# antonilo/unsupervised_detection

Hardware: NVIDIA H100
Metric: frame-pairs/sec adversarial train step 256x448 (higher is better)
Workload: dtype bf16

## Files before the change

### include/cis_b200.h

```cpp
#ifndef CIS_B200_H_
#define CIS_B200_H_
#include <stdint.h>
#include <stddef.h>

#ifdef __cplusplus
extern "C" {
#endif

typedef void* cis_stream_t;

enum { CIS_OK = 0, CIS_ERR_BAD_ARG = 1, CIS_ERR_UNSUPPORTED = 2, CIS_ERR_CUDA = 3 };
enum { CIS_ACT_NONE = 0, CIS_ACT_ELU = 1, CIS_ACT_LEAKY = 2 };
enum { CIS_MAX_TAPS = 49, CIS_MAX_SRC = 4 };

typedef struct {
  const void* ptr;
  int32_t pitch;
  int32_t c_off;
  int32_t chunks;
  int32_t n_mod;
} CisSrc;

typedef struct {
  int32_t N, H, W;
// ... 31 lines not shown
  int32_t ey, ex;
  int32_t splits;
  float* sk_scratch;
  int32_t* sk_counters;
  int32_t nph;
  int32_t ph_tap[5];
  int32_t sk_cluster;
  int32_t nsub;
  struct {
    int32_t tap0, ntaps;
    int32_t hoy, hox;
    int32_t OH, OW, oa, ob;
    const void* wpack;
  } sub[4];
  int32_t nwg;
} CisConv;

typedef struct {
  int32_t N, H, W, OH, OW, sh, sw, ntaps;
  int16_t dh[CIS_MAX_TAPS];
  int16_t dw[CIS_MAX_TAPS];
  int32_t nsrc;
  CisSrc src[CIS_MAX_SRC];
  const void* g;
  int32_t g_pitch, g_coff, g_chunks;
  float* dwp;
  int32_t Cout;
  int32_t K_pad;
  int32_t splits;
  int32_t tma;
// ... 115 lines not shown
```

### unsupervised_detection_b200/_lib.py

```python
import ctypes as C
import os

_HERE = os.path.dirname(os.path.abspath(__file__))
LIB_PATH = os.path.join(_HERE, os.environ.get('CIS_LIB_NAME', 'libcis_b200.so'))

MAX_TAPS, MAX_SRC = 49, 4
ACT_NONE, ACT_ELU, ACT_LEAKY = 0, 1, 2


class CisSrc(C.Structure):
    _fields_ = [('ptr', C.c_void_p), ('pitch', C.c_int32), ('c_off', C.c_int32), ('chunks', C.c_int32), ('n_mod', C.c_int32)]


class CisParamJob(C.Structure):
    _fields_ = [('kind', C.c_int32), ('i', C.c_int32 * 8), ('n', C.c_int64), ('p', C.c_void_p * 8)]


JOB_PACK, JOB_PACK_TILED, JOB_UNPACK, JOB_BN_FOLD, JOB_BN_CHAIN = range(5)


class CisSub(C.Structure):
    _fields_ = [('tap0', C.c_int32), ('ntaps', C.c_int32), ('hoy', C.c_int32), ('hox', C.c_int32), ('OH', C.c_int32), ('OW', C.c_int32),
                ('oa', C.c_int32), ('ob', C.c_int32), ('wpack', C.c_void_p)]

# ... 4 lines not shown
                ('dh', C.c_int16 * MAX_TAPS), ('dw', C.c_int16 * MAX_TAPS),
                ('nsrc', C.c_int32), ('src', CisSrc * MAX_SRC),
                ('wpack', C.c_void_p), ('K_pad', C.c_int32), ('BN', C.c_int32), ('n_tiles', C.c_int32),
                ('bias', C.c_void_p), ('act', C.c_int32), ('alpha', C.c_float),
                ('DH', C.c_int32), ('DW', C.c_int32), ('osh', C.c_int32), ('osw', C.c_int32), ('oa', C.c_int32), ('ob', C.c_int32),
                ('out', C.c_void_p), ('out_pitch', C.c_int32), ('out_coff', C.c_int32), ('out_ch', C.c_int32),
                ('outf', C.c_void_p), ('outf_pitch', C.c_int32), ('outf_coff', C.c_int32), ('outf_ch', C.c_int32),
                ('add_pre', C.c_void_p), ('add_pre_pitch', C.c_int32), ('add_pre_coff', C.c_int32),
                ('addf_pre', C.c_void_p), ('addf_pitch', C.c_int32), ('addf_coff', C.c_int32),
                ('add_post', C.c_void_p), ('add_post_pitch', C.c_int32), ('add_post_coff', C.c_int32),
                ('mode', C.c_int32),
                ('halo', C.c_int32), ('dil', C.c_int32), ('MT', C.c_int32), ('hoy', C.c_int32), ('hox', C.c_int32),
                ('ey', C.c_int32), ('ex', C.c_int32),
                ('splits', C.c_int32), ('sk_scratch', C.c_void_p), ('sk_counters', C.c_void_p),
                ('nph', C.c_int32), ('ph_tap', C.c_int32 * 5), ('sk_cluster', C.c_int32),
                ('nsub', C.c_int32), ('sub', CisSub * 4), ('nwg', C.c_int32)]


class CisWgrad(C.Structure):
    _fields_ = [('N', C.c_int32), ('H', C.c_int32), ('W', C.c_int32), ('OH', C.c_int32), ('OW', C.c_int32),
                ('sh', C.c_int32), ('sw', C.c_int32), ('ntaps', C.c_int32),
                ('dh', C.c_int16 * MAX_TAPS), ('dw', C.c_int16 * MAX_TAPS),
                ('nsrc', C.c_int32), ('src', CisSrc * MAX_SRC),
                ('g', C.c_void_p), ('g_pitch', C.c_int32), ('g_coff', C.c_int32), ('g_chunks', C.c_int32),
                ('dwp', C.c_void_p), ('Cout', C.c_int32), ('K_pad', C.c_int32), ('splits', C.c_int32), ('tma', C.c_int32),
                ('nh', C.c_int32), ('nwg', C.c_int32)]


_i32, _i64, _f32, _p, _u64 = C.c_int32, C.c_int64, C.c_float, C.c_void_p, C.c_uint64

_PROTOS = {
# ... 83 lines not shown
```

### unsupervised_detection_b200/csrc/conv_igemm.cu

```cuda
#include "ptx.cuh"
#include "../../include/cis_b200.h"
#include "common.cuh"
#include <cuda.h>
#include <stdlib.h>
#include <string.h>


namespace cis {

#ifdef CIS_TRACE
__device__ unsigned long long* g_trace = nullptr;
__device__ int g_trace_cap = 0;
#define CIS_TRACE_AT(slot)                                                                                         \
  do {                                                                                                             \
    if (g_trace && blockIdx.x == 0 && blockIdx.y == 0 && blockIdx.z == 0 && (slot) < g_trace_cap) g_trace[(slot)] = clock64(); \
  } while (0)
#else
#define CIS_TRACE_AT(slot) ((void)0)
#endif

static constexpr int kBM = 128;
static constexpr int kBK = 64;
static constexpr int kAStage = kBM * 128;
static constexpr int kThreads = 256;
// ... 522 lines not shown
__device__ __forceinline__ void halo_issue_any(const int nk16, float (&acc)[MTM][BN], const uint32_t hlo, const uint32_t blo, const uint32_t* s_aoff,
                                               const int gt, const int MT, const uint32_t ahi, const uint32_t bhi, const uint32_t a_mstep,
                                               const uint32_t a_half, const bool first) {
  static_assert(MTM >= 1 && MTM <= 4, "1..4 stacked tiles");
  if (MT == 1) halo_issue_nk<1>(nk16, acc, hlo, blo, s_aoff, gt, ahi, bhi, a_mstep, a_half, first);
  else if constexpr (MTM >= 2) {
    if (MT == 2) halo_issue_nk<2>(nk16, acc, hlo, blo, s_aoff, gt, ahi, bhi, a_mstep, a_half, first);
    else if constexpr (MTM >= 3) {
      if (MT == 3) halo_issue_nk<3>(nk16, acc, hlo, blo, s_aoff, gt, ahi, bhi, a_mstep, a_half, first);
      else if constexpr (MTM >= 4) halo_issue_nk<4>(nk16, acc, hlo, blo, s_aoff, gt, ahi, bhi, a_mstep, a_half, first);
    }
  }
  wg_wait<0>();
}

template <int BN, int NWG>
__global__ void __launch_bounds__(HaloCfg<BN, NWG>::kThreads, 1) conv_halo_kernel(const __grid_constant__ CisConv p, const int halo_stage_bytes, const int BS, const int NHS,
                                                        const __grid_constant__ HaloMaps maps, const int use_tma, const int G) {
  using Cfg = HaloCfg<BN, NWG>;
  constexpr int kBStage = BN * 128;
  constexpr int kHMmaWarp_ = Cfg::kMmaWarp, kHThreads_ = Cfg::kThreads;
  extern __shared__ uint8_t smem_raw[];
  __shared__ uint64_t bars[2 * 2 + 2 * kHaloMaxBStages + 1];
  __shared__ uint32_t s_aoff[CIS_MAX_TAPS];
  __shared__ SrcS s_src[CIS_MAX_SRC];

  const int tid = threadIdx.x, warp = tid >> 5, lane = tid & 31;
  const int MT = p.MT, MTC = NWG * MT, d = p.dil;
  const int nph = p.nph > 1 ? p.nph : 1;
  const int Wh = 8 + p.ex, Hh = 16 * MTC + p.ey, HP = Wh * Hh;
  const uint32_t stage_bytes = (uint32_t)G * kBStage;
  const uint32_t tile_base = (smem_u32(smem_raw) + 1023u) & ~1023u;
  const uint32_t h_base = tile_base;
  const uint32_t b_base = tile_base + NHS * halo_stage_bytes;
  int* pixtab = reinterpret_cast<int*>(smem_raw + (b_base + BS * stage_bytes - smem_u32(smem_raw)));
  const uint32_t bar_hfull = smem_u32(&bars[0]), bar_hempty = smem_u32(&bars[2]);
  const uint32_t bar_bfull = smem_u32(&bars[4]), bar_bempty = smem_u32(&bars[4 + kHaloMaxBStages]);
  const uint32_t bar_accum = smem_u32(&bars[4 + 2 * kHaloMaxBStages]);

  const bool grouped = p.nsub > 1;
  const int tap0 = grouped ? p.sub[blockIdx.z].tap0 : 0, ntaps = grouped ? p.sub[blockIdx.z].ntaps : p.ntaps;
  const int hoy = grouped ? p.sub[blockIdx.z].hoy : p.hoy, hox = grouped ? p.sub[blockIdx.z].hox : p.hox;
  const int OHs = grouped ? p.sub[blockIdx.z].OH : p.OH, OWs = grouped ? p.sub[blockIdx.z].OW : p.OW;
  const int oa = grouped ? p.sub[blockIdx.z].oa : p.oa, ob = grouped ? p.sub[blockIdx.z].ob : p.ob;
  const void* const wpack = grouped ? p.sub[blockIdx.z].wpack : p.wpack;
  const int Hp0 = (OHs + d - 1) / d, Wp0 = (OWs + d - 1) / d;
  const int tiles_x = (Wp0 + 7) / 8, tiles_y = (Hp0 + 16 * MTC - 1) / (16 * MTC);
  if (grouped && (int)blockIdx.x >= tiles_x * tiles_y * p.N) return;
  int bid = blockIdx.x;
  const int tx = bid % tiles_x; bid /= tiles_x;
  const int ty = bid % tiles_y; bid /= tiles_y;
  const int ph = bid % (d * d);
  const int n = bid / (d * d);
  const int pa = ph / d, pb = ph % d;
  const int ny = blockIdx.y;
  int m_chunks = 0;
  for (int i = 0; i < p.nsrc; ++i) m_chunks += p.src[i].chunks;
  const int nchunks_all = (m_chunks + 7) / 8;
  const int nsplit = (!grouped && p.splits > 1) ? p.splits : 1;
  const int cper = (nchunks_all + nsplit - 1) / nsplit;
  const int cc_lo = grouped ? 0 : blockIdx.z * cper;
  const int nchunks = min(cper, nchunks_all - cc_lo);
  __shared__ __align__(16) float s_bias[BN];
  pdl_launch_dependents();

  if (tid < ntaps) s_aoff[tid] = (uint32_t)((p.dh[tap0 + tid] * Wh + p.dw[tap0 + tid]) * 8);
  if (tid < p.nsrc) {
    s_src[tid].ptr = reinterpret_cast<const __nv_bfloat16*>(p.src[tid].ptr);
    s_src[tid].pitch = p.src[tid].pitch;
    s_src[tid].c_off = p.src[tid].c_off;
    s_src[tid].chunks = p.src[tid].chunks;
    s_src[tid].n_mod = p.src[tid].n_mod;
  }
  for (int q = tid; q < (use_tma ? 0 : HP); q += kHThreads_) {
    const int hy = q / Wh, hx = q - hy * Wh;
    const int gy = ty * 16 * MTC + hy + hoy, gx = tx * 8 + hx + hox;
    const int y = pa + d * gy, x = pb + d * gx;
    pixtab[q] = (gy >= 0 && gx >= 0 && y < p.H && x < p.W) ? (y * p.W + x) : -1;
  }
  if (tid == kHMmaWarp_ * 32) {
    for (int s = 0; s < 2; ++s) {
      mbar_init(bar_hfull + 8 * s, use_tma ? 1 : 96);
      mbar_init(bar_hempty + 8 * s, NWG);
    }
    for (int s = 0; s < BS; ++s) {
      mbar_init(bar_bfull + 8 * s, 1);
      mbar_init(bar_bempty + 8 * s, NWG);
    }
    mbar_init(bar_accum, 128 * NWG);
    fence_mbar_init();
  }
  if (use_tma && tid < p.nsrc) tma_prefetch_desc(&maps.m[tid]);
  pdl_wait();
  if (tid < BN) s_bias[tid] = p.bias ? p.bias[ny * BN + tid] : 0.f;
  __syncthreads();
  if (tid == 0) CIS_TRACE_AT(0);

  if (warp < kHMmaWarp_) {
// ... 1 lines not shown
    if (use_tma) {
      if (tid == 0) {
        int hcount = 0;
        for (int vc = 0; vc < nchunks * nph; ++vc) {
          const int cc = vc / nph, ph = vc - cc * nph;
          if (nph > 1 && p.ph_tap[ph + 1] == p.ph_tap[ph]) continue;
          const int hs = hcount % NHS;
          mbar_wait(bar_hempty + 8 * hs, (uint32_t)(((hcount / NHS) & 1) ^ 1));
          ++hcount;
          int c = (cc_lo + cc) * 8, si = 0;
          while (si < p.nsrc - 1 && c >= s_src[si].chunks) {
            c -= s_src[si].chunks;
            ++si;
          }
          const int nmod = s_src[si].n_mod;
          mbar_expect_tx(bar_hfull + 8 * hs, (uint32_t)(HP * 128));
          tma_load_4d(h_base + hs * halo_stage_bytes, &maps.m[si * nph + ph], bar_hfull + 8 * hs, c * 8, pb + d * (tx * 8 + hox),
                      pa + d * (ty * 16 * MTC + hoy), nmod ? (n % nmod) : n);
        }
      }
      __syncwarp();
    } else if (warp != 2) {
      const int hid = warp == 3 ? tid - 32 : tid;
      const int j = hid & 7, pl = hid >> 3;
      for (int cc = 0; cc < nchunks; ++cc) {
        const int hs = cc % NHS;
        mbar_wait(bar_hempty + 8 * hs, (uint32_t)(((cc / NHS) & 1) ^ 1));
        const int rem = m_chunks - (cc_lo + cc) * 8;
        const int nk16 = rem >= 8 ? 4 : (rem + 1) / 2;
        const bool need = j < 2 * nk16;
        const bool cvalid = j < rem;
        int c = (cc_lo + cc) * 8 + j, si = 0;
        if (cvalid) {
// ... 196 lines not shown
  if (!valid) return;
  float v[16];
  splitk_reduce16<BN>(tile0, nsplit, r, c0, v);
  epi_chunk(p, v, ny * BN + c0, dpix);
}
static constexpr int kPThreads = 448;
static constexpr int kPMaxAccCols = 64;

template <int BN>
__global__ void __launch_bounds__(kPThreads, 1) conv_halo_persist_kernel(const __grid_constant__ CisConv p, const int halo_stage_bytes,
                                                                       const int BS, const int NHS, const int AS, const int G,
                                                                       const __grid_constant__ HaloMaps maps, const int ws) {
  constexpr int kBStage = BN * 128;
  constexpr int kMaxHS = 4;
  extern __shared__ uint8_t smem_raw[];
  __shared__ uint64_t bars[2 * kMaxHS + 2 * kHaloMaxBStages + 4];
  __shared__ uint32_t s_aoff[CIS_MAX_TAPS];
  __shared__ __align__(16) float s_bias[BN];

  const int tid = threadIdx.x, warp = tid >> 5, lane = tid & 31;
  const int MT = p.MT;
  const int Wh = 8 + p.ex, Hh = 16 * MT + p.ey, HP = Wh * Hh;
  const uint32_t stage_bytes = (uint32_t)G * kBStage;
  const uint32_t tile_base = (smem_u32(smem_raw) + 1023u) & ~1023u;
  const uint32_t acc_bytes = (uint32_t)(MT * BN) * kAccColBytes;
  const uint32_t acc_base = tile_base, h_base = tile_base + AS * acc_bytes, b_base = h_base + NHS * halo_stage_bytes;
  const uint32_t bar_hfull = smem_u32(&bars[0]), bar_hempty = smem_u32(&bars[kMaxHS]);
  const uint32_t bar_bfull = smem_u32(&bars[2 * kMaxHS]), bar_bempty = smem_u32(&bars[2 * kMaxHS + kHaloMaxBStages]);
  const uint32_t bar_tfull = smem_u32(&bars[2 * kMaxHS + 2 * kHaloMaxBStages]), bar_tempty = smem_u32(&bars[2 * kMaxHS + 2 * kHaloMaxBStages + 2]);

  const int tiles_x = (p.OW + 7) / 8, tiles_y = (p.OH + 16 * MT - 1) / (16 * MT);
  const int total = tiles_x * tiles_y * p.N;
  int m_chunks = 0;
  for (int i = 0; i < p.nsrc; ++i) m_chunks += p.src[i].chunks;
  const int nchunks = (m_chunks + 7) / 8;

  pdl_launch_dependents();
  if (tid < p.ntaps) s_aoff[tid] = (uint32_t)((p.dh[tid] * Wh + p.dw[tid]) * 8);
  if (tid == 0) {
    for (int s = 0; s < NHS; ++s) {
      mbar_init(bar_hfull + 8 * s, 1);
      mbar_init(bar_hempty + 8 * s, 1);
    }
    for (int s = 0; s < BS; ++s) {
      mbar_init(bar_bfull + 8 * s, 1);
      mbar_init(bar_bempty + 8 * s, 1);
    }
    for (int s = 0; s < AS; ++s) {
      mbar_init(bar_tfull + 8 * s, 128);
      mbar_init(bar_tempty + 8 * s, 4);
    }
    fence_mbar_init();
  }
  if (tid < p.nsrc) tma_prefetch_desc(&maps.m[tid]);
  pdl_wait();
  if (tid < BN) s_bias[tid] = p.bias ? p.bias[tid] : 0.f;
  __syncthreads();
  if (tid == 0) {
    CIS_TRACE_AT(0);
    CIS_TRACE_AT(4);
  }

  if (warp == 12) {
    if (lane == 0) {
      int hs = 0;
      uint32_t hph = 1;
      for (int w = blockIdx.x; w < total; w += gridDim.x) {
        const int tx = w % tiles_x, r1 = w / tiles_x, ty = r1 % tiles_y, n = r1 / tiles_y;
        for (int cc = 0; cc < nchunks; ++cc) {
          mbar_wait(bar_hempty + 8 * hs, hph);
          int c = cc * 8, si = 0;
          while (si < p.nsrc - 1 && c >= p.src[si].chunks) {
            c -= p.src[si].chunks;
            ++si;
          }
          int nmod = p.src[0].n_mod;
          if (si == 1) nmod = p.src[1].n_mod;
          if (si == 2) nmod = p.src[2].n_mod;
          if (si == 3) nmod = p.src[3].n_mod;
          mbar_expect_tx(bar_hfull + 8 * hs, (uint32_t)(HP * 128));
          tma_load_4d(h_base + hs * halo_stage_bytes, &maps.m[si], bar_hfull + 8 * hs, c * 8, tx * 8 + p.hox, ty * 16 * MT + p.hoy,
                      nmod ? (n % nmod) : n);
          if (++hs == NHS) {
            hs = 0;
            hph ^= 1u;
          }
        }
      }
    }
  } else if (warp == 13) {
    if (lane == 0) {
      const uint8_t* wt = reinterpret_cast<const uint8_t*>(p.wpack);
      const int per_tile = nchunks * p.ntaps;
      if (ws) {
        if ((int)blockIdx.x < total) {
          mbar_expect_tx(bar_bfull, (uint32_t)(per_tile * kBStage));
          for (int it = 0; it < per_tile; it += 8) {
// ... 571 lines not shown
                           int estride = 1, int bc = 64, CUtensorMapSwizzle swz = CU_TENSOR_MAP_SWIZZLE_128B) {
  EncodeTiledFn enc = get_encode_tiled();
  if (!enc) return false;
  const int nb = s.n_mod > 0 ? s.n_mod : N;
  const int Hq = (H - py + step - 1) / step, Wq = (W - px + step - 1) / step;
  if (Hq < 1 || Wq < 1) return false;
  cuuint64_t dims[4] = {(cuuint64_t)s.chunks * 8, (cuuint64_t)Wq, (cuuint64_t)Hq, (cuuint64_t)nb};
  cuuint64_t strides[3] = {(cuuint64_t)step * s.pitch * 2, (cuuint64_t)step * W * s.pitch * 2, (cuuint64_t)H * W * s.pitch * 2};
  cuuint32_t box[4] = {(cuuint32_t)bc, (cuuint32_t)(bw * estride), (cuuint32_t)(bh * estride), 1};
  cuuint32_t es[4] = {1, (cuuint32_t)estride, (cuuint32_t)estride, 1};
  void* base = (void*)((const char*)s.ptr + ((size_t)(py * W + px) * s.pitch + (size_t)s.c_off) * 2);
  return enc(m, CU_TENSOR_MAP_DATA_TYPE_BFLOAT16, 4, base, dims, strides, box, es, CU_TENSOR_MAP_INTERLEAVE_NONE, swz,
             CU_TENSOR_MAP_L2_PROMOTION_L2_128B, CU_TENSOR_MAP_FLOAT_OOB_FILL_NONE) == CUDA_SUCCESS;
}

#ifdef CIS_TRACE
extern "C" int cis_trace_set(unsigned long long* buf, int cap) {
  cudaError_t e = cudaMemcpyToSymbol(cis::g_trace, &buf, sizeof(buf));
  if (e == cudaSuccess) e = cudaMemcpyToSymbol(cis::g_trace_cap, &cap, sizeof(cap));
  return e == cudaSuccess ? CIS_OK : cis_set_cuda_error(e, "cis_trace_set");
}
#endif

static int g_persist_mode = -1;
extern "C" int cis_set_persist_mode(int mode) {
  g_persist_mode = mode;
  return CIS_OK;
}

template <int BN, int NWG>
static int launch_halo(const CisConv* d, cudaStream_t st) {
  const int MTC = d->MT * NWG;
  const int Wh = 8 + d->ex, Hh = 16 * MTC + d->ey, HP = Wh * Hh;
  const int halo_stage = (HP * 128 + 1023) & ~1023;
  int chunks = 0;
  for (int i = 0; i < d->nsrc; ++i) chunks += d->src[i].chunks;
  const int nchunks = (chunks + 7) / 8;
  const int nsub = d->nsub > 1 ? d->nsub : 1;
  const int nsp = (nsub == 1 && d->splits > 1) ? d->splits : 1;
  const int cper = (nchunks + nsp - 1) / nsp;
  const int nhs = cper > 1 ? 2 : 1;
  const int dd = d->dil;
  int tiles = 0, ntaps_max = d->ntaps;
  if (nsub > 1) {
    if (nsub > 4 || dd != 1 || d->splits > 1 || d->nph > 1) return cis_set_error(CIS_ERR_BAD_ARG, "cis_conv_igemm(halo): bad grouped launch");
    ntaps_max = 0;
    int tsum = 0;
    for (int i = 0; i < nsub; ++i) {
      const int t = ((d->sub[i].OW + 7) / 8) * ((d->sub[i].OH + 16 * MTC - 1) / (16 * MTC));
      if (t > tiles) tiles = t;
      if (d->sub[i].ntaps > ntaps_max) ntaps_max = d->sub[i].ntaps;
// ... 39 lines not shown
  int splits = d->splits > 1 ? d->splits : 1;
  if (splits > 1) {
    const int per = (nchunks + splits - 1) / splits;
    if ((!d->sk_scratch && !d->sk_cluster) || d->sk_counters || (splits - 1) * per >= nchunks || (d->sk_cluster && splits > 8))
      return cis_set_error(CIS_ERR_BAD_ARG, "cis_conv_igemm(halo): bad split-K setup");
  }
  dim3 grid(tiles * dd * dd * d->N, d->n_tiles, nsub > 1 ? nsub : splits);
  HaloMaps maps;
  const int nph = d->nph > 1 ? d->nph : 1;
  static const int dil_tma = getenv("CIS_DIL_TMA") ? atoi(getenv("CIS_DIL_TMA")) : 1;
  int use_tma = ((d->dil == 1 || dil_tma) && Wh * d->dil <= 256 && Hh * d->dil <= 256) ? 1 : 0;
  for (int i = 0; use_tma && i < d->nsrc - 1; ++i)
    if (d->src[i].chunks % 8) use_tma = 0;
  for (int i = 0; use_tma && i < d->nsrc; ++i) {
    if (((uintptr_t)d->src[i].ptr + (size_t)d->src[i].c_off * 2) % 16) use_tma = 0;
    for (int ph = 0; use_tma && ph < nph; ++ph)
      if (!encode_src_map(&maps.m[i * nph + ph], d->src[i], d->N, d->H, d->W, Wh, Hh, nph > 1 ? 2 : 1, ph >> 1, ph & 1, d->dil)) use_tma = 0;
  }
  if (!use_tma) memset(&maps, 0, sizeof(maps));
  if (nph > 1 && !use_tma) return cis_set_error(CIS_ERR_UNSUPPORTED, "cis_conv_igemm(halo): stride-2 phases need the TMA halo path");
  const int persist_mode = g_persist_mode >= 0 ? g_persist_mode : (getenv("CIS_PERSIST_MODE") ? atoi(getenv("CIS_PERSIST_MODE")) : 1);
  static const int p_min_tiles = getenv("CIS_PERSIST_MIN_TILES") ? atoi(getenv("CIS_PERSIST_MIN_TILES")) : 296;
  static const int p_ws_kb = getenv("CIS_PERSIST_WS_KB") ? atoi(getenv("CIS_PERSIST_WS_KB")) : 112;
  if constexpr (BN <= kPMaxAccCols && NWG == 1) {
   if (persist_mode > 0 && use_tma && d->n_tiles == 1 && splits == 1 && nph == 1 && nsub == 1 && dd == 1 && d->MT * BN <= kPMaxAccCols) {
    const int total = tiles * d->N;
    const int per_tile = nchunks * d->ntaps;
    const int acc_stage = d->MT * BN * (int)kAccColBytes;
    const int AS = 2;
    const int fixed_p = AS * acc_stage + 1024;
    const int ws_bytes = per_tile * kB;
    int p_nhs = nchunks >= 3 ? 4 : 3;
    while (p_nhs > 2 && p_nhs * halo_stage + fixed_p + (ws_bytes <= p_ws_kb * 1024 ? ws_bytes : 2 * G * kB) > 226 * 1024) --p_nhs;
    const bool ws_fits = ws_bytes <= p_ws_kb * 1024 && p_nhs * halo_stage + fixed_p + ws_bytes <= 226 * 1024;
// ... 179 lines not shown
```

### unsupervised_detection_b200/engine.py

```python
import ctypes as C
import os

import numpy as np
import torch

from . import _lib
from ._lib import CisConv, CisWgrad, CisSrc, ACT_NONE, ACT_ELU, ACT_LEAKY


def ru(x, m):
    return (x + m - 1) // m * m


def same_pad(n_in, k, s=1, d=1):
    out = -(-n_in // s)
    total = max((out - 1) * s + (k - 1) * d + 1 - n_in, 0)
    return total // 2, total - total // 2


SIDE_STREAM = True
_SIDE = {}
MULTI_PARAM_OPS = os.environ.get('CIS_MULTI_PARAM', '1') == '1'
DACT_COLSUM = os.environ.get('CIS_DACT_COLSUM', '1') == '1'
PLAN_MODEL = int(os.environ.get('CIS_PLAN_MODEL', '4'))
# ... 138 lines not shown
                    n += 1
        return n

    def extend(self, other):
        self.ops += other.ops
        self.keep += other.keep


class Act(object):

    def __init__(self, N, H, W, C, device, buf=None, c_off=0, chanmap=None, n_mod=0, dep=frozenset(), name=''):
        if chanmap is not None and not C:
            C = max(chanmap) + 1
        self.N, self.H, self.W, self.C = N, H, W, C
        self.C8 = ru(C, 8) if chanmap is None else len(chanmap)
        if buf is None:
            buf = torch.zeros(N, H, W, self.C8, dtype=torch.bfloat16, device=device)
        self.buf = buf
        self.pitch = buf.shape[-1]
        self.c_off = c_off
        self.chanmap = list(chanmap) if chanmap is not None else list(range(C)) + [-1] * (self.C8 - C)
        self.n_mod = n_mod
        self.dep = frozenset(dep)
        self.name = name
        self.grad = None
        self.grad_written = {}
        self.device = device
        self.gen_rows = None

    @property
    def ptr(self):
        return self.buf.data_ptr()
# ... 97 lines not shown
    if cout > 64:
        return 64, 2, -(-npairs // p)
    nwg = 2 if npairs > p else 1
    return nh, nwg, -(-npairs // (nwg * p))




SPLITK = int(os.environ.get('CIS_SPLITK', '2'))
SPLITK_CLUSTER = os.environ.get('CIS_SPLITK_CLUSTER', '0') == '1'
SPLITK_MAX = int(os.environ.get('CIS_SPLITK_MAX', '16'))
SPLITK_NCTA = int(os.environ.get('CIS_SPLITK_NCTA', '64'))
SPLITK_MIN_UNITS = int(os.environ.get('CIS_SPLITK_MIN_UNITS', '18'))
HALO_SKIP_THIN = int(os.environ.get('CIS_HALO_SKIP_THIN', '0'))
HALO_MIN_UTIL = float(os.environ.get('CIS_HALO_MIN_UTIL', '0.2'))


HALO_NWG = int(os.environ.get('CIS_HALO_NWG', '2'))
HALO_NWG2_COST = 0.8


def halo_nwg(d, MT, Hp0, Wp0, dil, n_tiles, ntaps, nchunks, ey, ex):
    if HALO_NWG < 2 or d.BN < 64:
        return 1
    if HALO_NWG == 2 and n_tiles == 1 and dil == 1 and MT * d.BN <= 64 and nchunks * ntaps * d.BN * 128 <= 112 * 1024:
        return 1
    tiles_x = -(-Wp0 // 8)
    ty1, ty2 = -(-Hp0 // (16 * MT)), -(-Hp0 // (32 * MT))
    HP = (8 + ex) * (32 * MT + ey)
    nhs = 2 if nchunks > 1 else 1
# ... 29 lines not shown
    splits = min(units // min_units, -(-2 * NUM_SMS // ncta), SPLITK_MAX, 8 if SPLITK_CLUSTER else 1 << 30)
    if splits < 2:
        return
    per = -(-units // splits)
    splits = -(-units // per)
    if splits < 2:
        return
    if SPLITK_CLUSTER and splits <= 8 and mt * 128 * d.BN * 4 + 1024 <= 226 * 1024:
        d.splits, d.sk_scratch, d.sk_counters, d.sk_cluster = splits, None, None, 1
        return
    sc = torch.empty(ncta * mt * splits * 128 * d.BN, dtype=torch.float32, device=device)
    keep.append(sc)
    d.splits, d.sk_scratch, d.sk_counters = splits, sc.data_ptr(), None


def setup_halo(d, taps, dil, n_tiles):
    if not HALO_ENABLED or d.sh != 1 or d.sw != 1:
        return False
    if any(a % dil or b % dil for a, b in taps):
        return False
    if dil > 1 and (d.OH != d.H or d.OW != d.W):
        return False
    th = [(a // dil, b // dil) for a, b in taps]
    hoy, hox = min(a for a, _ in th), min(b for _, b in th)
    rel = [(a - hoy, b - hox) for a, b in th]
    ey, ex = max(a for a, _ in rel), max(b for _, b in rel)
    Hp0, Wp0 = -(-d.OH // dil), -(-d.OW // dil)
    tiles_x = -(-Wp0 // 8)
    best = None
    ntaps = len(taps)
    m_chunks = sum(d.src[i].chunks for i in range(d.nsrc))
    if HALO_SKIP_THIN and m_chunks * 8 <= HALO_SKIP_THIN and ntaps >= 16:
        return False
    nchunks = -(-m_chunks // 8)
    nhs = 2 if nchunks > 1 else 1
    force = int(os.environ.get('CIS_FORCE_MT128', '0')) if d.BN == 128 else 0
    for MT in (1, 2, 3, 4):
        if MT * d.BN > MAX_ACC_COLS or (force and MT != force):
            continue
        HP = (8 + ex) * (16 * MT + ey)
        fixed = nhs * ru(HP * 128, 1024) + HP * 4 + 1024
        smem = fixed + min(3, ntaps * nchunks) * d.BN * 128 + 1024
        if smem > 227 * 1024:
            continue
        tiles_y = -(-Hp0 // (16 * MT))
        util = (Hp0 * Wp0) / float(tiles_y * 16 * MT * tiles_x * 8)
        if util < (HALO_MIN_UTIL if dil == 1 else 0.5):
# ... 8 lines not shown
            per_sm = -(-ncta // NUM_SMS)
            cost = per_sm * max(t_mma, t_mem) + (4000.0 + 1500.0 * MT) * (-(-per_sm // cps))
        if PLAN_MODEL == 3:
            cost = float(MT)
        if PLAN_MODEL == 4:
            n1 = d.N * dil * dil * tiles_x * (-(-Hp0 // 16)) * n_tiles
            if not (2.0 * d.BN * ntaps * nchunks < 6000.0 and n1 > 4 * NUM_SMS):
                cost = float(MT)
        if best is None or cost < best[0] - 1e-9:
            best = (cost, MT, util)
    if best is None:
        return False
    d.halo, d.dil, d.MT, d.hoy, d.hox, d.ey, d.ex = 1, dil, best[1], hoy, hox, ey, ex
    d.nwg = halo_nwg(d, best[1], Hp0, Wp0, dil, n_tiles, ntaps, nchunks, ey, ex)
    _fill_taps(d, rel)
    return True


S2_HALO = os.environ.get('CIS_S2_HALO', '0') == '1'


def setup_halo_s2(d, taps, n_tiles):
    if not (HALO_ENABLED and S2_HALO) or d.sh != 2 or d.sw != 2:
        return None
    if any(d.src[i].chunks % 8 for i in range(d.nsrc - 1)):
        return None
    ph = [((u % 2) * 2 + (v % 2), u // 2, v // 2) for u, v in taps]
    order = sorted(range(len(taps)), key=lambda i: (ph[i][0], i))
    hoy, hox = min(a for _, a, _ in ph), min(b for _, _, b in ph)
    rel = [(ph[i][1] - hoy, ph[i][2] - hox) for i in order]
# ... 164 lines not shown
        kk = self.k * self.k
        if self.transposed:
            raise RuntimeError('use setup_transposed')
        kmap, Kp = self._kmap(range(kk), chanmap, self.cin * self.cout, self.cout)
        self.fwd_kmap, self.K_pad = kmap, Kp
        self.fwd_pack = torch.zeros(self.npad, Kp, dtype=torch.bfloat16, device=self.device)
        if self.bn:
            self.w_eff = torch.zeros(kk * self.cin * self.cout, dtype=torch.float32, device=self.device)
            self.b_eff = torch.zeros(self.npad, dtype=torch.float32, device=self.device)
            self.db_eff = torch.zeros(self.npad, dtype=torch.float32, device=self.device)

    def _alloc_tiles(self, ntaps, cin8, BN, n_tiles):
        nchunks = -(-cin8 // 64)
        return torch.zeros(n_tiles * nchunks * ntaps * BN * 64, dtype=torch.bfloat16, device=self.device)

    def fwd_tiles_buf(self, tap_order=None):
        if getattr(self, 'fwd_tiles', None) is None:
            self.fwd_tiles = self._alloc_tiles(self.k * self.k, len(self.in_chanmap), self.BN, self.n_tiles)
            self.fwd_tiles_kmap = self.fwd_kmap
            if tap_order is not None:
                self.fwd_tiles_kmap, _ = self._kmap(list(tap_order), self.in_chanmap, self.cin * self.cout, self.cout)
            self.fwd_tap_order = tap_order
        assert getattr(self, 'fwd_tap_order', None) == tap_order, self.name
        return self.fwd_tiles

    def w_src_ptr(self):
        return self.w_eff.data_ptr() if self.bn else self.store.ptr(self.wkey)

    def bias_ptr(self):
        return self.b_eff.data_ptr() if self.bn else self.store.ptr(self.bkey)

# ... 3 lines not shown
            plan.add('cis_bn_fold', s.ptr(self.wkey), s.ptr(self.bkey), s.ptr(self.name + '/gamma'), s.ptr(self.name + '/beta'),
                     self.k * self.k * self.cin * self.cout, self.cout, self.w_eff.data_ptr(), self.b_eff.data_ptr())
        if self.fwd_pack is not None:
            if self.transposed:
                for pk in self.tr_packs:
                    if pk.get('wt') is not None:
                        plan.add('cis_pack_weights_tiled', self.w_src_ptr(), pk['kmap'].data_ptr(), len(self.in_chanmap), len(pk['taps']),
                                 self.n_tiles, self.BN, self.cout, self.cin, None, pk['wt'].data_ptr())
                    if pk.get('rows_used', True):
                        plan.add('cis_pack_weights', self.w_src_ptr(), pk['kmap'].data_ptr(), pk['K_pad'], self.npad, self.cout, self.cin,
                                 None, pk['w'].data_ptr())
            else:
                if getattr(self, 'fwd_tiles', None) is not None:
                    plan.add('cis_pack_weights_tiled', self.w_src_ptr(), self.fwd_tiles_kmap.data_ptr(), len(self.in_chanmap), self.k * self.k,
                             self.n_tiles, self.BN, self.cout, 1, None, self.fwd_tiles.data_ptr())
                if getattr(self, 'fwd_rows_used', True):
                    plan.add('cis_pack_weights', self.w_src_ptr(), self.fwd_kmap.data_ptr(), self.K_pad, self.npad, self.cout, 1,
                             None, self.fwd_pack.data_ptr())
        if dgrad and self.dgrad_packs:
            cout8 = ru(self.cout, 8)
            for pk in self.dgrad_packs:
                if pk.get('wt') is not None:
                    plan.add('cis_pack_weights_tiled', self.w_src_ptr(), pk['kmap'].data_ptr(), cout8, len(pk['taps']), pk['n_tiles'], pk['BN'],
                             len(self.in_chanmap), self.cout, pk['nmap'].data_ptr(), pk['wt'].data_ptr())
                if pk.get('rows_used', True):
                    plan.add('cis_pack_weights', self.w_src_ptr(), pk['kmap'].data_ptr(), pk['K_pad'], pk['rows'], len(self.in_chanmap),
                             self.cout, pk['nmap'].data_ptr(), pk['w'].data_ptr())

    def plan_finalize(self, bp, mode):
        if not hasattr(self, 'dwp') or mode not in getattr(self, 'wg_splits', {}):
            return
        s = self.store
        bp.add('cis_unpack_wgrad', self.dwp.data_ptr(), self.wg_kmap.data_ptr(), self.wg_K_pad, self.cout, self.wg_splits[mode],
               s.ptr(self.wkey, 'grad'), self.colpart.data_ptr(), self.col_blocks[mode], self.cout,
               (self.db_eff.data_ptr() if self.bn else s.ptr(self.bkey, 'grad')), 0 if self.wg_halo else 1)
        if self.bn:
            bp.add('cis_bn_chain', s.ptr(self.wkey), s.ptr(self.bkey), s.ptr(self.name + '/gamma'), s.ptr(self.wkey, 'grad'),
                   self.db_eff.data_ptr(), self.k * self.k * self.cin * self.cout, self.cout, s.ptr(self.bkey, 'grad'),
                   s.ptr(self.name + '/gamma', 'grad'), s.ptr(self.name + '/beta', 'grad'))
# ... 115 lines not shown
        if out is not None:
            d.out, d.out_pitch, d.out_coff, d.out_ch = out.ptr, out.pitch, out.c_off, out.C8
        if outf is not None:
            d.outf, d.outf_pitch, d.outf_coff, d.outf_ch = outf.data_ptr(), outf.shape[-1], 0, outf_ch or outf.shape[-1]
        if addf is not None:
            d.addf_pre, d.addf_pitch, d.addf_coff = addf.data_ptr(), addf.shape[-1], 0
            if outf is None:
                d.outf_ch = addf.shape[-1]
        if post_add is not None:
            d.add_post, d.add_post_pitch, d.add_post_coff = post_add.ptr, post_add.pitch, post_add.c_off
        d.mode = mode
        order = setup_halo_s2(d, taps, layer.n_tiles) if (layer.stride == 2 and layer.dil == 1) else None
        if order is not None:
            d.wpack = layer.fwd_tiles_buf(order).data_ptr()
            layer.fwd_rows_used = getattr(layer, 'fwd_rows_used', False)
        elif layer.stride == 1 and setup_halo(d, taps, layer.dil, layer.n_tiles):
            d.wpack = layer.fwd_tiles_buf().data_ptr()
            layer.fwd_rows_used = getattr(layer, 'fwd_rows_used', False)
        else:
            layer.fwd_rows_used = True
        setup_splitk(d, self.device, plan.keep)
        plan.keep.append(d)
        plan.keep += [srcs, out, outf, addf, post_add, layer]
        plan.add('cis_conv_igemm', C.byref(d), flops=2.0 * N * OH * OW * layer.k * layer.k * layer.cin * layer.cout, lane=self.lane)
        if layer.tag:
            self.tape.append(lambda bp, m, L=layer, S=list(srcs), O=out, P=post_add: self._conv_bwd(bp, m, L, S, O, P))
        return out

    def _conv_bwd(self, bp, mode, layer, srcs, out, post_add):
        if out is None or mode not in out.dep or not out.grad_written.get(mode):
            return
        G = out.get_grad()
# ... 92 lines not shown
            oh = -(-(H - pk['a']) // s)
            ow = -(-(W - pk['b']) // s)
            if oh <= 0 or ow <= 0:
                continue
            d = CisConv()
            d.N, d.H, d.W, d.OH, d.OW, d.sh, d.sw = nb, out.H, out.W, oh, ow, 1, 1
            _fill_taps(d, pk['taps'])
            d.nsrc = 1
            d.src[0] = G.src()
            d.wpack, d.K_pad, d.BN, d.n_tiles = pk['w'].data_ptr(), pk['K_pad'], pk['BN'], pk['n_tiles']
            d.bias, d.act = None, ACT_NONE
            d.DH, d.DW, d.osh, d.osw, d.oa, d.ob = H, W, s, s, pk['a'], pk['b']
            d.out, d.out_pitch, d.out_coff, d.out_ch = tgt.ptr, tgt.pitch, tgt.c_off, tgt.C8
            if acc:
                d.add_pre, d.add_pre_pitch, d.add_pre_coff = tgt.ptr, tgt.pitch, tgt.c_off
            if setup_halo(d, pk['taps'], layer.dil if s == 1 else 1, pk['n_tiles']):
                if pk.get('wt') is None:
                    pk['wt'] = layer._alloc_tiles(len(pk['taps']), ru(layer.cout, 8), pk['BN'], pk['n_tiles'])
                d.wpack = pk['wt'].data_ptr()
                pk['rows_used'] = pk.get('rows_used', False)
            else:
                pk['rows_used'] = True
            emitted.append((d, 2.0 * nb * oh * ow * len(pk['taps']) * layer.cin * layer.cout))
        grp = merge_parity_launches([d for d, _ in emitted]) if len(emitted) > 1 else None
        if grp is not None:
            bp.keep.append(grp)
            bp.add('cis_conv_igemm', C.byref(grp), flops=sum(f for _, f in emitted))
        else:
            for d, fl in emitted:
                setup_splitk(d, self.device, bp.keep)
                bp.keep.append(d)
# ... 150 lines not shown
```

Measured before the change: 619.8.

## Fold adjacent horizontal taps into 64-channel K chunks for thin-channel halo convs

For stride-1 convolutions whose single source has 8, 16 or 32 channels, the halo conv kernel now treats f adjacent pixels as one 64-wide channel chunk, loaded by a TMA map with an offset base. This merges groups of horizontal taps into one K step, cutting the number of MMA steps and the wasted padding for thin-channel layers. Edge tiles get a warp fixup pass that zeroes out-of-image pixels before the consumer barrier is released. New folded weight-pack buffers and guard-padded activation allocations are added, which adds pack work and extra sync on edge tiles.

Result: no change. 625.9 (median of 6 runs) (+1.0%).

```diff
diff --git a/include/cis_b200.h b/include/cis_b200.h
--- a/include/cis_b200.h
+++ b/include/cis_b200.h
@@ -69,6 +69,7 @@
     const void* wpack;
   } sub[4];
   int32_t nwg;
+  int32_t fold;
 } CisConv;
 
 typedef struct {
diff --git a/unsupervised_detection_b200/_lib.py b/unsupervised_detection_b200/_lib.py
--- a/unsupervised_detection_b200/_lib.py
+++ b/unsupervised_detection_b200/_lib.py
@@ -42,7 +42,7 @@
                 ('ey', C.c_int32), ('ex', C.c_int32),
                 ('splits', C.c_int32), ('sk_scratch', C.c_void_p), ('sk_counters', C.c_void_p),
                 ('nph', C.c_int32), ('ph_tap', C.c_int32 * 5), ('sk_cluster', C.c_int32),
-                ('nsub', C.c_int32), ('sub', CisSub * 4), ('nwg', C.c_int32)]
+                ('nsub', C.c_int32), ('sub', CisSub * 4), ('nwg', C.c_int32), ('fold', C.c_int32)]
 
 
 class CisWgrad(C.Structure):
diff --git a/unsupervised_detection_b200/csrc/conv_igemm.cu b/unsupervised_detection_b200/csrc/conv_igemm.cu
--- a/unsupervised_detection_b200/csrc/conv_igemm.cu
+++ b/unsupervised_detection_b200/csrc/conv_igemm.cu
@@ -560,6 +560,24 @@
   wg_wait<0>();
 }
 
+__device__ __forceinline__ bool fold_edge(int x0, int Wh, int f, int W) { return x0 < 0 || x0 + Wh + f - 2 >= W; }
+__device__ __forceinline__ void fold_fixup(uint32_t h, int x0, int Wh, int Hh, int f, int W, int lane) {
+  const int gsh = f == 8 ? 0 : (f == 4 ? 1 : 2);
+  const int L = min(Wh, max(0, -x0));
+  const int R0 = min(Wh, max(L, W - x0 - f + 1));
+  const int nb = L + (Wh - R0);
+  const int j = lane & 7;
+  for (int k = 0; k < nb; ++k) {
+    const int hx = k < L ? k : R0 + (k - L);
+    const int pix = x0 + hx + (j >> gsh);
+    if (pix >= 0 && pix < W) continue;
+    for (int hy = lane >> 3; hy < Hh; hy += 4) {
+      const int q = hy * Wh + hx;
+      asm volatile("st.shared.v4.u32 [%0], {%1, %1, %1, %1};" ::"r"(h + (uint32_t)(q * 128) + (uint32_t)((j ^ (q & 7)) << 4)), "r"(0) : "memory");
+    }
+  }
+}
+
 template <int BN, int NWG>
 __global__ void __launch_bounds__(HaloCfg<BN, NWG>::kThreads, 1) conv_halo_kernel(const __grid_constant__ CisConv p, const int halo_stage_bytes, const int BS, const int NHS,
                                                         const __grid_constant__ HaloMaps maps, const int use_tma, const int G) {
@@ -567,7 +585,7 @@
   constexpr int kBStage = BN * 128;
   constexpr int kHMmaWarp_ = Cfg::kMmaWarp, kHThreads_ = Cfg::kThreads;
   extern __shared__ uint8_t smem_raw[];
-  __shared__ uint64_t bars[2 * 2 + 2 * kHaloMaxBStages + 1];
+  __shared__ uint64_t bars[2 * 2 + 2 * kHaloMaxBStages + 1 + 2];
   __shared__ uint32_t s_aoff[CIS_MAX_TAPS];
   __shared__ SrcS s_src[CIS_MAX_SRC];
 
@@ -583,6 +601,7 @@
   const uint32_t bar_hfull = smem_u32(&bars[0]), bar_hempty = smem_u32(&bars[2]);
   const uint32_t bar_bfull = smem_u32(&bars[4]), bar_bempty = smem_u32(&bars[4 + kHaloMaxBStages]);
   const uint32_t bar_accum = smem_u32(&bars[4 + 2 * kHaloMaxBStages]);
+  const uint32_t bar_hraw = smem_u32(&bars[5 + 2 * kHaloMaxBStages]);
 
   const bool grouped = p.nsub > 1;
   const int tap0 = grouped ? p.sub[blockIdx.z].tap0 : 0, ntaps = grouped ? p.sub[blockIdx.z].ntaps : p.ntaps;
@@ -600,9 +619,12 @@
   const int n = bid / (d * d);
   const int pa = ph / d, pb = ph % d;
   const int ny = blockIdx.y;
+  const int fold = p.fold > 1 ? p.fold : 1;
   int m_chunks = 0;
   for (int i = 0; i < p.nsrc; ++i) m_chunks += p.src[i].chunks;
+  if (fold > 1) m_chunks = 8;
   const int nchunks_all = (m_chunks + 7) / 8;
+  const bool fix = fold > 1 && fold_edge(tx * 8 + hox, Wh, fold, p.W);
   const int nsplit = (!grouped && p.splits > 1) ? p.splits : 1;
   const int cper = (nchunks_all + nsplit - 1) / nsplit;
   const int cc_lo = grouped ? 0 : blockIdx.z * cper;
@@ -628,6 +650,7 @@
     for (int s = 0; s < 2; ++s) {
       mbar_init(bar_hfull + 8 * s, use_tma ? 1 : 96);
       mbar_init(bar_hempty + 8 * s, NWG);
+      mbar_init(bar_hraw + 8 * s, 1);
     }
     for (int s = 0; s < BS; ++s) {
       mbar_init(bar_bfull + 8 * s, 1);
@@ -659,9 +682,19 @@
             ++si;
           }
           const int nmod = s_src[si].n_mod;
-          mbar_expect_tx(bar_hfull + 8 * hs, (uint32_t)(HP * 128));
-          tma_load_4d(h_base + hs * halo_stage_bytes, &maps.m[si * nph + ph], bar_hfull + 8 * hs, c * 8, pb + d * (tx * 8 + hox),
+          const uint32_t bar = (fix ? bar_hraw : bar_hfull) + 8 * hs;
+          mbar_expect_tx(bar, (uint32_t)(HP * 128));
+          tma_load_4d(h_base + hs * halo_stage_bytes, &maps.m[si * nph + ph], bar, c * 8, fold > 1 ? tx * 8 : pb + d * (tx * 8 + hox),
                       pa + d * (ty * 16 * MTC + hoy), nmod ? (n % nmod) : n);
+        }
+      } else if (warp == 1 && fix) {
+        for (int cc = 0; cc < nchunks; ++cc) {
+          const int hs = cc % NHS;
+          mbar_wait(bar_hraw + 8 * hs, (uint32_t)((cc / NHS) & 1));
+          fold_fixup(h_base + hs * halo_stage_bytes, tx * 8 + hox, Wh, Hh, fold, p.W, lane);
+          fence_proxy_async();
+          __syncwarp();
+          if (lane == 0) mbar_arrive(bar_hfull + 8 * hs);
         }
       }
       __syncwarp();
@@ -888,7 +921,7 @@
   constexpr int kBStage = BN * 128;
   constexpr int kMaxHS = 4;
   extern __shared__ uint8_t smem_raw[];
-  __shared__ uint64_t bars[2 * kMaxHS + 2 * kHaloMaxBStages + 4];
+  __shared__ uint64_t bars[3 * kMaxHS + 2 * kHaloMaxBStages + 4];
   __shared__ uint32_t s_aoff[CIS_MAX_TAPS];
   __shared__ __align__(16) float s_bias[BN];
 
@@ -902,11 +935,14 @@
   const uint32_t bar_hfull = smem_u32(&bars[0]), bar_hempty = smem_u32(&bars[kMaxHS]);
   const uint32_t bar_bfull = smem_u32(&bars[2 * kMaxHS]), bar_bempty = smem_u32(&bars[2 * kMaxHS + kHaloMaxBStages]);
   const uint32_t bar_tfull = smem_u32(&bars[2 * kMaxHS + 2 * kHaloMaxBStages]), bar_tempty = smem_u32(&bars[2 * kMaxHS + 2 * kHaloMaxBStages + 2]);
+  const uint32_t bar_hraw = smem_u32(&bars[2 * kMaxHS + 2 * kHaloMaxBStages + 4]);
+  const int fold = p.fold > 1 ? p.fold : 1;
 
   const int tiles_x = (p.OW + 7) / 8, tiles_y = (p.OH + 16 * MT - 1) / (16 * MT);
   const int total = tiles_x * tiles_y * p.N;
   int m_chunks = 0;
   for (int i = 0; i < p.nsrc; ++i) m_chunks += p.src[i].chunks;
+  if (fold > 1) m_chunks = 8;
   const int nchunks = (m_chunks + 7) / 8;
 
   pdl_launch_dependents();
@@ -915,6 +951,7 @@
     for (int s = 0; s < NHS; ++s) {
       mbar_init(bar_hfull + 8 * s, 1);
       mbar_init(bar_hempty + 8 * s, 1);
+      mbar_init(bar_hraw + 8 * s, 1);
     }
     for (int s = 0; s < BS; ++s) {
       mbar_init(bar_bfull + 8 * s, 1);
@@ -936,25 +973,38 @@
   }
 
   if (warp == 12) {
-    if (lane == 0) {
+    {
       int hs = 0;
-      uint32_t hph = 1;
+      uint32_t hph = 1, rawph = 0;
       for (int w = blockIdx.x; w < total; w += gridDim.x) {
         const int tx = w % tiles_x, r1 = w / tiles_x, ty = r1 % tiles_y, n = r1 / tiles_y;
+        const bool fix = fold > 1 && fold_edge(tx * 8 + p.hox, Wh, fold, p.W);
         for (int cc = 0; cc < nchunks; ++cc) {
-          mbar_wait(bar_hempty + 8 * hs, hph);
-          int c = cc * 8, si = 0;
-          while (si < p.nsrc - 1 && c >= p.src[si].chunks) {
-            c -= p.src[si].chunks;
-            ++si;
+          if (lane == 0) {
+            mbar_wait(bar_hempty + 8 * hs, hph);
+            int c = cc * 8, si = 0;
+            while (si < p.nsrc - 1 && c >= p.src[si].chunks) {
+              c -= p.src[si].chunks;
+              ++si;
+            }
+            int nmod = p.src[0].n_mod;
+            if (si == 1) nmod = p.src[1].n_mod;
+            if (si == 2) nmod = p.src[2].n_mod;
+            if (si == 3) nmod = p.src[3].n_mod;
+            const uint32_t bar = (fix ? bar_hraw : bar_hfull) + 8 * hs;
+            mbar_expect_tx(bar, (uint32_t)(HP * 128));
+            tma_load_4d(h_base + hs * halo_stage_bytes, &maps.m[si], bar, c * 8, fold > 1 ? tx * 8 : tx * 8 + p.hox, ty * 16 * MT + p.hoy,
+                        nmod ? (n % nmod) : n);
           }
-          int nmod = p.src[0].n_mod;
-          if (si == 1) nmod = p.src[1].n_mod;
-          if (si == 2) nmod = p.src[2].n_mod;
-          if (si == 3) nmod = p.src[3].n_mod;
-          mbar_expect_tx(bar_hfull + 8 * hs, (uint32_t)(HP * 128));
-          tma_load_4d(h_base + hs * halo_stage_bytes, &maps.m[si], bar_hfull + 8 * hs, c * 8, tx * 8 + p.hox, ty * 16 * MT + p.hoy,
-                      nmod ? (n % nmod) : n);
+          if (fix) {
+            mbar_wait(bar_hraw + 8 * hs, (rawph >> hs) & 1u);
+            rawph ^= 1u << hs;
+            fold_fixup(h_base + hs * halo_stage_bytes, tx * 8 + p.hox, Wh, Hh, fold, p.W, lane);
+            fence_proxy_async();
+            __syncwarp();
+            if (lane == 0) mbar_arrive(bar_hfull + 8 * hs);
+          }
+          __syncwarp();
           if (++hs == NHS) {
             hs = 0;
             hph ^= 1u;
@@ -1556,6 +1606,19 @@
              CU_TENSOR_MAP_L2_PROMOTION_L2_128B, CU_TENSOR_MAP_FLOAT_OOB_FILL_NONE) == CUDA_SUCCESS;
 }
 
+static bool encode_fold_map(CUtensorMap* m, const CisSrc& s, int N, int H, int W, int bw, int bh, int x0) {
+  EncodeTiledFn enc = get_encode_tiled();
+  if (!enc) return false;
+  const int nb = s.n_mod > 0 ? s.n_mod : N;
+  cuuint64_t dims[4] = {64, (cuuint64_t)(W + x0), (cuuint64_t)H, (cuuint64_t)nb};
+  cuuint64_t strides[3] = {(cuuint64_t)s.pitch * 2, (cuuint64_t)W * s.pitch * 2, (cuuint64_t)H * W * s.pitch * 2};
+  cuuint32_t box[4] = {64, (cuuint32_t)bw, (cuuint32_t)bh, 1};
+  cuuint32_t es[4] = {1, 1, 1, 1};
+  void* base = (void*)((const char*)s.ptr - (ptrdiff_t)x0 * s.pitch * 2);
+  return enc(m, CU_TENSOR_MAP_DATA_TYPE_BFLOAT16, 4, base, dims, strides, box, es, CU_TENSOR_MAP_INTERLEAVE_NONE, CU_TENSOR_MAP_SWIZZLE_128B,
+             CU_TENSOR_MAP_L2_PROMOTION_L2_128B, CU_TENSOR_MAP_FLOAT_OOB_FILL_NONE) == CUDA_SUCCESS;
+}
+
 #ifdef CIS_TRACE
 extern "C" int cis_trace_set(unsigned long long* buf, int cap) {
   cudaError_t e = cudaMemcpyToSymbol(cis::g_trace, &buf, sizeof(buf));
@@ -1577,6 +1640,14 @@
   const int halo_stage = (HP * 128 + 1023) & ~1023;
   int chunks = 0;
   for (int i = 0; i < d->nsrc; ++i) chunks += d->src[i].chunks;
+  const int fold = d->fold > 1 ? d->fold : 1;
+  if (fold > 1) {
+    const CisSrc& s0 = d->src[0];
+    if (d->nsrc != 1 || d->nsub > 1 || d->nph > 1 || d->dil != 1 || d->splits > 1 || s0.c_off != 0 || s0.chunks * 8 != s0.pitch ||
+        s0.pitch * fold != 64 || d->hox > 0 || d->ex % fold)
+      return cis_set_error(CIS_ERR_BAD_ARG, "cis_conv_igemm(halo): bad folded launch");
+    chunks = 8;
+  }
   const int nchunks = (chunks + 7) / 8;
   const int nsub = d->nsub > 1 ? d->nsub : 1;
   const int nsp = (nsub == 1 && d->splits > 1) ? d->splits : 1;
@@ -1646,10 +1717,15 @@
     if (d->src[i].chunks % 8) use_tma = 0;
   for (int i = 0; use_tma && i < d->nsrc; ++i) {
     if (((uintptr_t)d->src[i].ptr + (size_t)d->src[i].c_off * 2) % 16) use_tma = 0;
+    if (fold > 1) {
+      if (use_tma && !encode_fold_map(&maps.m[0], d->src[0], d->N, d->H, d->W, Wh, Hh, -d->hox)) use_tma = 0;
+      continue;
+    }
     for (int ph = 0; use_tma && ph < nph; ++ph)
       if (!encode_src_map(&maps.m[i * nph + ph], d->src[i], d->N, d->H, d->W, Wh, Hh, nph > 1 ? 2 : 1, ph >> 1, ph & 1, d->dil)) use_tma = 0;
   }
   if (!use_tma) memset(&maps, 0, sizeof(maps));
+  if (fold > 1 && !use_tma) return cis_set_error(CIS_ERR_UNSUPPORTED, "cis_conv_igemm(halo): folded launch needs its TMA map");
   if (nph > 1 && !use_tma) return cis_set_error(CIS_ERR_UNSUPPORTED, "cis_conv_igemm(halo): stride-2 phases need the TMA halo path");
   const int persist_mode = g_persist_mode >= 0 ? g_persist_mode : (getenv("CIS_PERSIST_MODE") ? atoi(getenv("CIS_PERSIST_MODE")) : 1);
   static const int p_min_tiles = getenv("CIS_PERSIST_MIN_TILES") ? atoi(getenv("CIS_PERSIST_MIN_TILES")) : 296;
diff --git a/unsupervised_detection_b200/engine.py b/unsupervised_detection_b200/engine.py
--- a/unsupervised_detection_b200/engine.py
+++ b/unsupervised_detection_b200/engine.py
@@ -176,8 +176,13 @@
             C = max(chanmap) + 1
         self.N, self.H, self.W, self.C = N, H, W, C
         self.C8 = ru(C, 8) if chanmap is None else len(chanmap)
+        self.fold_guard = buf is None and self.C8 in FOLD_PITCHES
         if buf is None:
-            buf = torch.zeros(N, H, W, self.C8, dtype=torch.bfloat16, device=device)
+            if self.fold_guard:
+                flat = torch.zeros(N * H * W * self.C8 + 2 * FOLD_GUARD, dtype=torch.bfloat16, device=device)
+                buf = flat[FOLD_GUARD:FOLD_GUARD + N * H * W * self.C8].view(N, H, W, self.C8)
+            else:
+                buf = torch.zeros(N, H, W, self.C8, dtype=torch.bfloat16, device=device)
         self.buf = buf
         self.pitch = buf.shape[-1]
         self.c_off = c_off
@@ -305,6 +310,12 @@
 SPLITK_MIN_UNITS = int(os.environ.get('CIS_SPLITK_MIN_UNITS', '18'))
 HALO_SKIP_THIN = int(os.environ.get('CIS_HALO_SKIP_THIN', '0'))
 HALO_MIN_UTIL = float(os.environ.get('CIS_HALO_MIN_UTIL', '0.2'))
+HALO_FOLD = os.environ.get('CIS_HALO_FOLD', '1') != '0'
+FOLD_PITCHES = (8, 16, 32)
+FOLD_MIN_TAPS = 8
+FOLD_MIN_COLS = 512
+FOLD_MIN_CTAS = NUM_SMS
+FOLD_GUARD = 256
 
 
 HALO_NWG = int(os.environ.get('CIS_HALO_NWG', '2'))
@@ -364,7 +375,42 @@
     d.splits, d.sk_scratch, d.sk_counters = splits, sc.data_ptr(), None
 
 
-def setup_halo(d, taps, dil, n_tiles):
+def halo_fold(d, rel, dil):
+    if not HALO_FOLD or dil != 1 or d.nsrc != 1:
+        return None
+    s = d.src[0]
+    P = s.chunks * 8
+    if s.c_off != 0 or s.pitch != P or P not in FOLD_PITCHES:
+        return None
+    kh, kw = max(a for a, _ in rel) + 1, max(b for _, b in rel) + 1
+    if kw < 2 or sorted(rel) != [(a, b) for a in range(kh) for b in range(kw)]:
+        return None
+    f = 64 // P
+    nf = kh * (-(-kw // f))
+    if len(rel) - nf < FOLD_MIN_TAPS or (len(rel) - nf) * d.BN * d.n_tiles < FOLD_MIN_COLS:
+        return None
+    if d.N * (-(-d.OW // 8)) * (-(-d.OH // 16)) * d.n_tiles < FOLD_MIN_CTAS:
+        return None
+    index = {t: i for i, t in enumerate(rel)}
+    folded, groups = [], []
+    for a in range(kh):
+        for b0 in range(0, kw, f):
+            folded.append((a, b0))
+            groups.append([index.get((a, b0 + j)) for j in range(f)])
+    return f, folded, groups
+
+
+def fold_kmap(kmap, m, groups):
+    km = kmap.cpu().numpy()
+    out = np.full(len(groups) * 64, -1, dtype=np.int32)
+    for t, grp in enumerate(groups):
+        for j, ti in enumerate(grp):
+            if ti is not None:
+                out[t * 64 + j * m:t * 64 + (j + 1) * m] = km[ti * m:(ti + 1) * m]
+    return torch.from_numpy(out).to(kmap.device)
+
+
+def setup_halo(d, taps, dil, n_tiles, fold_ok=False):
     if not HALO_ENABLED or d.sh != 1 or d.sw != 1:
         return False
     if any(a % dil or b % dil for a, b in taps):
@@ -374,13 +420,16 @@
     th = [(a // dil, b // dil) for a, b in taps]
     hoy, hox = min(a for a, _ in th), min(b for _, b in th)
     rel = [(a - hoy, b - hox) for a, b in th]
+    fold = halo_fold(d, rel, dil) if fold_ok else None
+    if fold is not None:
+        rel = fold[1]
     ey, ex = max(a for a, _ in rel), max(b for _, b in rel)
     Hp0, Wp0 = -(-d.OH // dil), -(-d.OW // dil)
     tiles_x = -(-Wp0 // 8)
     best = None
-    ntaps = len(taps)
+    ntaps = len(rel)
     m_chunks = sum(d.src[i].chunks for i in range(d.nsrc))
-    if HALO_SKIP_THIN and m_chunks * 8 <= HALO_SKIP_THIN and ntaps >= 16:
+    if HALO_SKIP_THIN and m_chunks * 8 <= HALO_SKIP_THIN and len(taps) >= 16:
         return False
     nchunks = -(-m_chunks // 8)
     nhs = 2 if nchunks > 1 else 1
@@ -419,6 +468,9 @@
     d.halo, d.dil, d.MT, d.hoy, d.hox, d.ey, d.ex = 1, dil, best[1], hoy, hox, ey, ex
     d.nwg = halo_nwg(d, best[1], Hp0, Wp0, dil, n_tiles, ntaps, nchunks, ey, ex)
     _fill_taps(d, rel)
+    if fold is not None:
+        d.fold = fold[0]
+        return fold[2]
     return True
 
 
@@ -613,7 +665,13 @@
         nchunks = -(-cin8 // 64)
         return torch.zeros(n_tiles * nchunks * ntaps * BN * 64, dtype=torch.bfloat16, device=self.device)
 
-    def fwd_tiles_buf(self, tap_order=None):
+    def fwd_tiles_buf(self, tap_order=None, fold=None):
+        if fold is not None:
+            if getattr(self, 'fwd_tiles_fold', None) is None:
+                self.fwd_tiles_fold = self._alloc_tiles(len(fold), 64, self.BN, self.n_tiles)
+                self.fwd_fold_kmap, self.fwd_fold_groups = fold_kmap(self.fwd_kmap, len(self.in_chanmap), fold), fold
+            assert self.fwd_fold_groups == fold, self.name
+            return self.fwd_tiles_fold
         if getattr(self, 'fwd_tiles', None) is None:
             self.fwd_tiles = self._alloc_tiles(self.k * self.k, len(self.in_chanmap), self.BN, self.n_tiles)
             self.fwd_tiles_kmap = self.fwd_kmap
@@ -647,6 +705,9 @@
                 if getattr(self, 'fwd_tiles', None) is not None:
                     plan.add('cis_pack_weights_tiled', self.w_src_ptr(), self.fwd_tiles_kmap.data_ptr(), len(self.in_chanmap), self.k * self.k,
                              self.n_tiles, self.BN, self.cout, 1, None, self.fwd_tiles.data_ptr())
+                if getattr(self, 'fwd_tiles_fold', None) is not None:
+                    plan.add('cis_pack_weights_tiled', self.w_src_ptr(), self.fwd_fold_kmap.data_ptr(), 64, len(self.fwd_fold_groups),
+                             self.n_tiles, self.BN, self.cout, 1, None, self.fwd_tiles_fold.data_ptr())
                 if getattr(self, 'fwd_rows_used', True):
                     plan.add('cis_pack_weights', self.w_src_ptr(), self.fwd_kmap.data_ptr(), self.K_pad, self.npad, self.cout, 1,
                              None, self.fwd_pack.data_ptr())
@@ -656,6 +717,9 @@
                 if pk.get('wt') is not None:
                     plan.add('cis_pack_weights_tiled', self.w_src_ptr(), pk['kmap'].data_ptr(), cout8, len(pk['taps']), pk['n_tiles'], pk['BN'],
                              len(self.in_chanmap), self.cout, pk['nmap'].data_ptr(), pk['wt'].data_ptr())
+                if pk.get('wtf') is not None:
+                    plan.add('cis_pack_weights_tiled', self.w_src_ptr(), pk['wtf_kmap'].data_ptr(), 64, len(pk['wtf_groups']), pk['n_tiles'],
+                             pk['BN'], len(self.in_chanmap), self.cout, pk['nmap'].data_ptr(), pk['wtf'].data_ptr())
                 if pk.get('rows_used', True):
                     plan.add('cis_pack_weights', self.w_src_ptr(), pk['kmap'].data_ptr(), pk['K_pad'], pk['rows'], len(self.in_chanmap),
                              self.cout, pk['nmap'].data_ptr(), pk['w'].data_ptr())
@@ -801,8 +865,8 @@
         if order is not None:
             d.wpack = layer.fwd_tiles_buf(order).data_ptr()
             layer.fwd_rows_used = getattr(layer, 'fwd_rows_used', False)
-        elif layer.stride == 1 and setup_halo(d, taps, layer.dil, layer.n_tiles):
-            d.wpack = layer.fwd_tiles_buf().data_ptr()
+        elif layer.stride == 1 and (hr := setup_halo(d, taps, layer.dil, layer.n_tiles, fold_ok=len(srcs) == 1 and srcs[0].fold_guard)):
+            d.wpack = layer.fwd_tiles_buf(fold=hr if d.fold > 1 else None).data_ptr()
             layer.fwd_rows_used = getattr(layer, 'fwd_rows_used', False)
         else:
             layer.fwd_rows_used = True
@@ -925,7 +989,15 @@
             d.out, d.out_pitch, d.out_coff, d.out_ch = tgt.ptr, tgt.pitch, tgt.c_off, tgt.C8
             if acc:
                 d.add_pre, d.add_pre_pitch, d.add_pre_coff = tgt.ptr, tgt.pitch, tgt.c_off
-            if setup_halo(d, pk['taps'], layer.dil if s == 1 else 1, pk['n_tiles']):
+            hr = setup_halo(d, pk['taps'], layer.dil if s == 1 else 1, pk['n_tiles'], fold_ok=s == 1 and G.fold_guard)
+            if hr and d.fold > 1:
+                if pk.get('wtf') is None:
+                    pk['wtf'] = layer._alloc_tiles(len(hr), 64, pk['BN'], pk['n_tiles'])
+                    pk['wtf_kmap'], pk['wtf_groups'] = fold_kmap(pk['kmap'], ru(layer.cout, 8), hr), hr
+                assert pk['wtf_groups'] == hr, layer.name
+                d.wpack = pk['wtf'].data_ptr()
+                pk['rows_used'] = pk.get('rows_used', False)
+            elif hr:
                 if pk.get('wt') is None:
                     pk['wt'] = layer._alloc_tiles(len(pk['taps']), ru(layer.cout, 8), pk['BN'], pk['n_tiles'])
                 d.wpack = pk['wt'].data_ptr()
```
